# ChuhanZhou/News_Recommendation_Model

Hardware: AMD Instinct MI355X
Metric: train impressions/sec (higher is better)
Workload: dtype f32

## Files before the change

### include/nrm_hotpath.h

```cpp
#ifndef NRM_HOTPATH_H
#define NRM_HOTPATH_H

#ifdef __cplusplus
extern "C" {
#endif

#define NRM_ABI_VERSION 7
#define NRM_OK 0
#define NRM_EINVAL (-1)
#define NRM_ELAUNCH (-2)

typedef void* nrm_stream_t;

int nrm_abi_version(void);
const char* nrm_last_error(void);
int nrm_build_flags(void);
const char* nrm_source_digest(void);
const char* nrm_build_info(void);


#define NRM_MMA_F32 0
#define NRM_MMA_BF16 1
#define NRM_MMA_BF16X3 2
long nrm_pwattn_packed_floats(int D);
// ... 59 lines not shown
    const float* ws; int nsplit, nj, ldws, ni;
    float* out; long out_istride, out_jstride;
    float* out2; long out2_istride, out2_jstride; float sign2;
    const float* vec; float* vec_out;
} nrm_slab_desc;
int nrm_slab_reduce_multi(const nrm_slab_desc* descs, int n, nrm_stream_t stream);

int nrm_head_fold(const float* w_o1, const float* b_o1, const float* w_m2, const float* b_m2, int P, int Q, int R,
                  float* packed_fwd, float* packed_bwd, float* bias, nrm_stream_t stream);
int nrm_head_fold_bwd(const float* dwp, int ldp, const float* dbp, const float* w_o1, const float* w_m2, const float* b_m2,
                      int P, int Q, int R, float* dw_o1, float* dw_m2, float* db_o1, float* db_m2, nrm_stream_t stream);

int nrm_colreduce(int mode, const float* x, const float* dy, const float* mean, const float* rstd,
                  float* s0, float* s1, int R, int N, int ld, nrm_stream_t stream);
int nrm_bn_finalize(int stage, const float* s, float* out, float* running, int R, int N, float momentum, float eps,
                    nrm_stream_t stream);
int nrm_mul_bwd(const float* dy, int lddy, const float* g, int ldg, const float* e, int lde, float* dg, float* de, int ldo,
                int R, int N, nrm_stream_t stream);
int nrm_bn_apply(const float* x, const float* mean, const float* rstd, const float* gamma, const float* beta,
                 float* y, int R, int N, int ld, nrm_stream_t stream);
int nrm_bn_backward(const float* x, const float* dy, const float* mean, const float* rstd, const float* gamma,
                    const float* s0, const float* s1, const float* add, float* dx, int R, int N, int ld, int training,
                    nrm_stream_t stream);
int nrm_concat_cols(const float* const* srcs, const long* lds, const int* widths, int n, float* out, int ldo, long R,
                    nrm_stream_t stream);

int nrm_pool_bmm(const float* W, long wsb, long wsi, long wsj, const float* X, int ldx, float* out,
                 int B, int I, int J, int D, int accumulate, nrm_stream_t stream);
int nrm_pool_rowdot(const float* g, int ldg, const float* h, float* ds, int B, int T, int H, int D, float* zero_out, int zero_n,
                    nrm_stream_t stream);

int nrm_small_linear_relu_fwd(const void* x, int x_is_f64, const float* weight, const float* bias, float* y, long R, int K, int N, int ldy,
                              nrm_stream_t stream);
int nrm_small_linear_relu_bwd(const void* x, int x_is_f64, const float* weight, const float* bias, const float* dy, int lddy, long R,
                              int K, int N, float* dwb, nrm_stream_t stream);

int nrm_loss_fwd_bwd(const float* out, int out_stride, const void* label, int label_is_f64, const long* user_id, const float* delta,
                     long n_delta, float alpha, int B, int T, float* loss_sum, float* dout, int dout_stride, float* ddelta, int* err,
                     nrm_stream_t stream);

int nrm_adam_step(float* p, float* g, float* m, float* v, long n, float lr, float beta1, float beta2, float eps,
                  float weight_decay, int step, int zero_grad, nrm_stream_t stream);
int nrm_gather_flat(const float* const* srcs, const long* offsets, const long* counts, int n, float* flat, long flat_n,
                    nrm_stream_t stream);
int nrm_adam_step_dev(float* p, float* g, float* m, float* v, long n, float lr, float beta1, float beta2, float eps,
                      float weight_decay, float* state, int zero_grad, nrm_stream_t stream);

int nrm_frontend_fwd(const void* x, int x_is_f64, int nrows, int xcols, int P, int n_sub, int behaviour,
                     const float* cat_tab, int n_cat, int e0, const float* sen_w, const float* sen_b, int e1,
                     const float* type_tab, int n_type, int e2,
                     const float* year_tab, const float* month_tab, const float* day_tab, const float* hour_tab,
                     int n_year, int n_month, int n_day, int n_hour, int e3,
                     float* lab, int ldlab, float* ti, int ldti, int* err, nrm_stream_t stream);
int nrm_frontend_bwd(const void* x, int x_is_f64, int nrows, int xcols, int P, int n_sub, int behaviour,
                     const float* dlab, int lddl, const float* sen_w, const float* sen_b,
                     int n_cat, int e0, int e1, int n_type, int e2, int n_year, int n_month, int n_day, int n_hour, int e3,
                     float* d_cat_tab, float* d_sen_w, float* d_sen_b, float* d_type_tab,
                     float* d_year_tab, float* d_month_tab, float* d_day_tab, float* d_hour_tab, nrm_stream_t stream);

long nrm_frontend_tables_ws_floats(long nrows_total, int n_sub, int e1, int n_type, int e2, int n_year, int n_month, int n_day, int n_hour, int e3);
int nrm_frontend_bwd_tables(const void* x0, int nrows0, int xcols0, int behaviour0, const float* dlab0, int lddl0,
                            const void* x1, int nrows1, int xcols1, int behaviour1, const float* dlab1, int lddl1, int x_is_f64,
                            int P, int n_sub, const float* sen_w, const float* sen_b,
                            int e0, int e1, int n_type, int e2, int n_year, int n_month, int n_day, int n_hour, int e3,
                            float* d_sen_w, float* d_sen_b, float* d_type_tab,
                            float* d_year_tab, float* d_month_tab, float* d_day_tab, float* d_hour_tab, float* ws, nrm_stream_t stream);

long nrm_frontend_cat_ws_ints(int n_cat, long nrows_total, int n_sub);
int nrm_frontend_cat_grad(const void* x0, int nrows0, int xcols0, const float* dlab0, int lddl0,
                          const void* x1, int nrows1, int xcols1, const float* dlab1, int lddl1, int x_is_f64,
                          int P, int n_sub, int n_cat, int e0, float* d_cat_tab, int* ws, nrm_stream_t stream);

int nrm_row_auc(const float* score, const float* label, const int* len, int B, int T, float* auc, int* top1,
                nrm_stream_t stream);

int nrm_ensemble_rank_max_candidates(void);
int nrm_ensemble_rank(const float* const* logits, const long* row_stride, const long* col_stride, int M, const int* empty,
                      const float* label, int B, int T, float* score, int* rank, int* live, float* metrics, nrm_stream_t stream);

int nrm_compact_gather(const void* x_target, int target_cols, int target_is_f64, const void* x_global, int global_cols, int global_is_f64,
                       const int* cand_off, const int* pad_mult, int B, int T, int trim, int N,
                       void* xt_compact, void* xg_compact, int* flag, nrm_stream_t stream);
int nrm_pwattn_fwd_ragged(const float* t, const float* h, const float* u, const float* v, const float* packed_wp,
                          const float* w2, const float* b2, float* s, const int* cand_imp, const int* cand_off,
                          int B, int N, int max_count, int H, int D, int mma, nrm_stream_t stream);
int nrm_pool_bmm_ragged(const float* s, const float* h, float* out, const int* cand_off, int B, int N, int max_count, int H, int D,
                        nrm_stream_t stream);
int nrm_ensemble_rank_ragged(const float* const* logits, const long* col_stride, int M, const int* cand_off, const int* pad_mult, int N,
                             const float* label, int B, int T, float* score, int* rank, int* live, float* metrics, nrm_stream_t stream);

int nrm_history_len(const void* x_history, int cols, int is_f64, int B, int H, int* hist_len, nrm_stream_t stream);
int nrm_history_gather(const void* x_history, int cols, int is_f64, const int* hist_off, int B, int H, int R, int k_max, void* xh_compact,
                       nrm_stream_t stream);
int nrm_history_tiles(const int* cand_imp, const int* cand_off, const int* hist_off, const int* tile_pre, int B, int N, int R, int Mt,
                      void* tile_tab, nrm_stream_t stream);
int nrm_pwattn_fwd_hragged(const float* t, const float* h, const float* u, const float* v, const float* packed_wp,
                           const float* w2, const float* b2, float* s, const int* cand_imp, const int* cand_off, const int* hist_off,
                           const int* tile_pre, const void* tile_tab, int B, int N, int max_count, int R, int Mt, int k_max, int D, int mma,
                           nrm_stream_t stream);
int nrm_pool_bmm_hragged(const float* s, const float* h, float* out, const int* cand_off, const int* hist_off, const int* hist_mult,
                         const int* tile_pre, int B, int N, int max_count, int R, int Mt, int k_max, int D, nrm_stream_t stream);

#define NRM_PWATTN_FWD_FORM_LEN 18
#define NRM_FWD_STREAM 0
#define NRM_FWD_RW_TILE 1
#define NRM_FWD_WALK_BF16 2
// ... 58 lines not shown
```

### news_recommendation_model_amd/csrc/capi.hip

```cpp
#include <stdarg.h>
#include <stdint.h>
#include <stdio.h>
#include <stdlib.h>
#include <vector>

#include "../../include/nrm_hotpath.h"
#include "common.hpp"
#include "pwattn.hpp"
#include "gemm.hpp"
#include "head.hpp"
#include "pool_loss.hpp"
#include "frontend.hpp"
#include "scoring.hpp"
#include "compact.hpp"
#include "assemble.hpp"
#include "epoch.hpp"

static thread_local char g_err[512] = "";

static int fail(int code, const char* fmt, ...) {
    va_list ap;
    va_start(ap, fmt);
    vsnprintf(g_err, sizeof(g_err), fmt, ap);
    va_end(ap);
// ... 831 lines not shown
    nrm::EnsembleLogits lg = {};
    for (int m = 0; m < M; ++m) {
        if (!logits[m] && N > 0) return fail(NRM_EINVAL, "nrm_ensemble_rank_ragged: logits[%d] is a null pointer", m);
        const long cs = col_stride ? col_stride[m] : 1;
        if (cs < 1) return fail(NRM_EINVAL, "nrm_ensemble_rank_ragged: model %d has entry stride %ld (need >= 1)", m, cs);
        lg.ptr[m] = logits[m]; lg.row_stride[m] = 0; lg.col_stride[m] = cs;
    }
    return check_hip(nrm::ensemble_rank_ragged_launch(lg, M, cand_off, pad_mult, N, label, B, T, score, rank, live, metrics, (hipStream_t)stream),
                     "ensemble_rank_ragged");
}

int nrm_compact_gather(const void* x_target, int target_cols, int target_is_f64, const void* x_global, int global_cols, int global_is_f64,
                       const int* cand_off, const int* pad_mult, int B, int T, int trim, int N,
                       void* xt_compact, void* xg_compact, int* flag, nrm_stream_t stream) {
    if (B < 0 || T <= 0 || trim < 0 || trim > T || N < 0 || target_cols <= 0 || global_cols <= 0)
        return fail(NRM_EINVAL, "nrm_compact_gather: B=%d T=%d trim=%d N=%d target_cols=%d global_cols=%d", B, T, trim, N, target_cols, global_cols);
    if ((long)N > (long)B * (T - trim)) return fail(NRM_EINVAL, "nrm_compact_gather: N=%d compact rows exceed the B*(T - trim)=%ld kept cells", N, (long)B * (T - trim));
    if (!cand_off || !pad_mult || !flag || !x_target || !x_global || (N > 0 && (!xt_compact || !xg_compact))) return fail(NRM_EINVAL, "nrm_compact_gather: null pointer");
    nrm::CompactGatherParams p;
    p.xt = (const unsigned*)x_target; p.xg = (const unsigned*)x_global; p.xt_c = (unsigned*)xt_compact; p.xg_c = (unsigned*)xg_compact;
    p.wt = target_cols * (target_is_f64 ? 2 : 1); p.wg = global_cols * (global_is_f64 ? 2 : 1);
    p.cand_off = cand_off; p.pad_mult = pad_mult; p.B = B; p.T = T; p.Tp = T - trim; p.N = N; p.flag = flag;
    return check_hip(nrm::compact_gather_launch(p, (hipStream_t)stream), "compact_gather");
}

static int check_fe(const char* fn, int nrows, int xcols, int P, int n_sub, int behaviour, int e0, int e1, int e2, int e3) {
    if (nrows < 0 || P <= 0 || n_sub < 0 || e0 <= 0 || e1 <= 0 || e2 <= 0 || e3 <= 0)
        return fail(NRM_EINVAL, "%s: bad dimension", fn);
    if (n_sub > 16) return fail(NRM_EINVAL, "%s: n_sub=%d (<= 16 sub-category slots)", fn, n_sub);
    const int need = 4 + P + 1 + n_sub + 3 + 1 + (behaviour ? 2 : 0);
    if (xcols < need) return fail(NRM_EINVAL, "%s: packed rows have %d columns, layout needs %d", fn, xcols, need);
    return NRM_OK;
}

int nrm_frontend_fwd(const void* x, int x_is_f64, int nrows, int xcols, int P, int n_sub, int behaviour,
                     const float* cat_tab, int n_cat, int e0, const float* sen_w, const float* sen_b, int e1,
                     const float* type_tab, int n_type, int e2,
                     const float* year_tab, const float* month_tab, const float* day_tab, const float* hour_tab,
                     int n_year, int n_month, int n_day, int n_hour, int e3,
                     float* lab, int ldlab, float* ti, int ldti, int* err, nrm_stream_t stream) {
    if (int rc = check_fe("nrm_frontend_fwd", nrows, xcols, P, n_sub, behaviour, e0, e1, e2, e3)) return rc;
    if (!x || !cat_tab || !sen_w || !sen_b || !type_tab || !year_tab || !month_tab || !day_tab || !hour_tab || !lab || !ti || !err)
        return fail(NRM_EINVAL, "nrm_frontend_fwd: null pointer");
    if (ldlab < e0 + e1 + e2 + e3 + (behaviour ? 2 : 0) || ldti < P) return fail(NRM_EINVAL, "nrm_frontend_fwd: ldlab=%d ldti=%d too small", ldlab, ldti);
    nrm::FrontendParams p = {};
    p.cat_tab = cat_tab; p.sen_w = sen_w; p.sen_b = sen_b; p.type_tab = type_tab;
    p.year_tab = year_tab; p.month_tab = month_tab; p.day_tab = day_tab; p.hour_tab = hour_tab;
    p.n_cat = n_cat; p.n_type = n_type; p.n_year = n_year; p.n_month = n_month; p.n_day = n_day; p.n_hour = n_hour;
    p.e0 = e0; p.e1 = e1; p.e2 = e2; p.e3 = e3; p.P = P; p.n_sub = n_sub; p.xcols = xcols; p.behaviour = behaviour;
    p.lab = lab; p.ldlab = ldlab; p.ti = ti; p.ldti = ldti; p.err = err;
    return check_hip(nrm::frontend_fwd_launch(p, x, x_is_f64, nrows, (hipStream_t)stream), "frontend_fwd");
}

int nrm_frontend_bwd(const void* x, int x_is_f64, int nrows, int xcols, int P, int n_sub, int behaviour,
                     const float* dlab, int lddl, const float* sen_w, const float* sen_b,
                     int n_cat, int e0, int e1, int n_type, int e2, int n_year, int n_month, int n_day, int n_hour, int e3,
                     float* d_cat_tab, float* d_sen_w, float* d_sen_b, float* d_type_tab,
                     float* d_year_tab, float* d_month_tab, float* d_day_tab, float* d_hour_tab, nrm_stream_t stream) {
    if (int rc = check_fe("nrm_frontend_bwd", nrows, xcols, P, n_sub, behaviour, e0, e1, e2, e3)) return rc;
    const int n_small = !!d_sen_w + !!d_sen_b + !!d_type_tab + !!d_year_tab + !!d_month_tab + !!d_day_tab + !!d_hour_tab;
    if (!x || !dlab || !sen_w || !sen_b || (n_small != 7 && (n_small != 0 || !d_cat_tab)))
        return fail(NRM_EINVAL, "nrm_frontend_bwd: null pointer");
    if (lddl < e0 + e1 + e2 + e3) return fail(NRM_EINVAL, "nrm_frontend_bwd: lddl=%d too small", lddl);
    nrm::FrontendParams p = {};
    p.sen_w = sen_w; p.sen_b = sen_b;
    p.d_cat_tab = d_cat_tab; p.d_sen_w = d_sen_w; p.d_sen_b = d_sen_b; p.d_type_tab = d_type_tab;
    p.d_year_tab = d_year_tab; p.d_month_tab = d_month_tab; p.d_day_tab = d_day_tab; p.d_hour_tab = d_hour_tab;
    p.n_cat = n_cat; p.n_type = n_type; p.n_year = n_year; p.n_month = n_month; p.n_day = n_day; p.n_hour = n_hour;
    p.e0 = e0; p.e1 = e1; p.e2 = e2; p.e3 = e3; p.P = P; p.n_sub = n_sub; p.xcols = xcols; p.behaviour = behaviour;
    return check_hip(nrm::frontend_bwd_launch(p, x, x_is_f64, dlab, lddl, nrows, (hipStream_t)stream), "frontend_bwd");
}

static nrm::FrontendParams tab_dims(int n_sub, int e1, int n_type, int e2, int n_year, int n_month, int n_day, int n_hour, int e3) {
    nrm::FrontendParams p = {};
    p.n_type = n_type; p.n_year = n_year; p.n_month = n_month; p.n_day = n_day; p.n_hour = n_hour;
    p.e1 = e1; p.e2 = e2; p.e3 = e3; p.n_sub = n_sub;
    return p;
}

long nrm_frontend_tables_ws_floats(long nrows_total, int n_sub, int e1, int n_type, int e2, int n_year, int n_month, int n_day, int n_hour, int e3) {
    if (nrows_total <= 0 || n_sub < 0) return 0;
    return nrm::tab_grad_ws_floats(tab_dims(n_sub, e1, n_type, e2, n_year, n_month, n_day, n_hour, e3), nrows_total);
}

int nrm_frontend_bwd_tables(const void* x0, int nrows0, int xcols0, int behaviour0, const float* dlab0, int lddl0,
                            const void* x1, int nrows1, int xcols1, int behaviour1, const float* dlab1, int lddl1, int x_is_f64,
                            int P, int n_sub, const float* sen_w, const float* sen_b,
                            int e0, int e1, int n_type, int e2, int n_year, int n_month, int n_day, int n_hour, int e3,
                            float* d_sen_w, float* d_sen_b, float* d_type_tab,
                            float* d_year_tab, float* d_month_tab, float* d_day_tab, float* d_hour_tab, float* ws, nrm_stream_t stream) {
    if (nrows0 > 0) if (int rc = check_fe("nrm_frontend_bwd_tables", nrows0, xcols0, P, n_sub, behaviour0, e0, e1, e2, e3)) return rc;
    if (nrows1 > 0) if (int rc = check_fe("nrm_frontend_bwd_tables", nrows1, xcols1, P, n_sub, behaviour1, e0, e1, e2, e3)) return rc;
    if (nrows0 < 0 || nrows1 < 0 || (long)nrows0 + nrows1 >= (1L << 31) - 64) return fail(NRM_EINVAL, "nrm_frontend_bwd_tables: nrows=%d,%d", nrows0, nrows1);
    if ((nrows0 > 0 && (!x0 || !dlab0 || lddl0 < e0 + e1 + e2 + e3)) || (nrows1 > 0 && (!x1 || !dlab1 || lddl1 < e0 + e1 + e2 + e3)))
        return fail(NRM_EINVAL, "nrm_frontend_bwd_tables: null pointer or lddl too small");
    if (!sen_w || !sen_b || !d_sen_w || !d_sen_b || !d_type_tab || !d_year_tab || !d_month_tab || !d_day_tab || !d_hour_tab || !ws)
        return fail(NRM_EINVAL, "nrm_frontend_bwd_tables: null pointer");
    nrm::FrontendParams p = tab_dims(n_sub, e1, n_type, e2, n_year, n_month, n_day, n_hour, e3);
    p.e0 = e0; p.P = P; p.n_cat = 1;
    p.sen_w = sen_w; p.sen_b = sen_b;
    p.d_sen_w = d_sen_w; p.d_sen_b = d_sen_b; p.d_type_tab = d_type_tab;
    p.d_year_tab = d_year_tab; p.d_month_tab = d_month_tab; p.d_day_tab = d_day_tab; p.d_hour_tab = d_hour_tab;
    if (nrm::tab_grad_ws_floats(p, (long)nrows0 + nrows1) <= 0 && nrows0 + nrows1 > 0)
        return fail(NRM_EINVAL, "nrm_frontend_bwd_tables: shape not taken (nrm_frontend_tables_ws_floats is 0): use nrm_frontend_bwd");
    return check_hip(nrm::tab_grad_launch(p, x0, nrows0, xcols0, dlab0, lddl0, x1, nrows1, xcols1, dlab1, lddl1, x_is_f64, ws,
                                          (hipStream_t)stream), "frontend_bwd_tables");
// ... 101 lines not shown
```

### news_recommendation_model_amd/csrc/frontend.hip

```cpp
#include <algorithm>
#include "common.hpp"
#include "frontend.hpp"

namespace nrm {

template <typename XT>
__device__ __forceinline__ int row_index(const XT* xr, int col, int limit, int* err) {
    const int i = (int)xr[col];
    if (i < 0 || i >= limit) { *err = 1; return i < 0 ? 0 : limit - 1; }
    return i;
}

constexpr int FE_MAXSUB = 16;
constexpr int FE_HDR = 6 + FE_MAXSUB;
struct RowHeaders {
    int* idx;
    float* sen;
};

template <typename XT>
__device__ __forceinline__ void stage_headers(const FrontendParams& p, int xcols, int* err, const XT* __restrict__ x, int r_lo, int nr,
                                              const RowHeaders& hd, int nthreads) {
    const int P = p.P, NS = p.n_sub;
    const int c_cat = 4 + P, c_sub = c_cat + 1, c_sen = c_sub + NS, c_typ = c_sen + 3;
    const int items = 9 + NS;
    for (int i = threadIdx.x; i < nr * items; i += nthreads) {
        const int r = i / items, k = i - r * items;
        const XT* xr = x + (size_t)(r_lo + r) * xcols;
        if (k < 4) {
            const int lim = k == 0 ? p.n_year : k == 1 ? p.n_month : k == 2 ? p.n_day : p.n_hour;
            hd.idx[r * FE_HDR + k] = row_index(xr, k, lim, err);
        } else if (k == 4) {
            hd.idx[r * FE_HDR + 4] = row_index(xr, c_cat, p.n_cat, err);
        } else if (k == 5) {
            hd.idx[r * FE_HDR + 5] = row_index(xr, c_typ, p.n_type, err);
        } else if (k < 6 + NS) {
            hd.idx[r * FE_HDR + k] = row_index(xr, c_sub + (k - 6), p.n_cat, err);
        } else {
            hd.sen[r * 4 + (k - 6 - NS)] = (float)xr[c_sen + (k - 6 - NS)];
        }
    }
}

constexpr int FWD_ROWS = 8;
constexpr int FE_THREADS = 256;

template <typename XT>
__global__ __launch_bounds__(FE_THREADS) void frontend_fwd_kernel(const FrontendParams p, const XT* __restrict__ x, int nrows) {
    __shared__ int h_idx[FWD_ROWS * FE_HDR];
    __shared__ float h_sen[FWD_ROWS * 4];
    const int r_lo = blockIdx.x * FWD_ROWS, nr = min(FWD_ROWS, nrows - r_lo);
    const RowHeaders hd = {h_idx, h_sen};
    stage_headers(p, p.xcols, p.err, x, r_lo, nr, hd, FE_THREADS);
    __syncthreads();
    const int P = p.P, NS = p.n_sub;
    const int c_beh = 4 + P + 1 + NS + 3 + 1;
    const int e0 = p.e0, e1 = p.e1, e2 = p.e2, e3 = p.e3;
    const int width = e0 + e1 + e2 + e3 + (p.behaviour ? 2 : 0);
    const float inv_ns = 1.0f / (float)NS;
    float* lab = p.lab + (size_t)r_lo * p.ldlab;
    for (int i = threadIdx.x; i < nr * p.ldlab; i += FE_THREADS) {
        const int r = i / p.ldlab, c = i - r * p.ldlab;
        const int* hi = h_idx + r * FE_HDR;
        float v = 0.f;
        if (c < e0) {
            float sub = 0.f;
            for (int k = 0; k < NS; ++k) sub += p.cat_tab[(size_t)hi[6 + k] * e0 + c];
            v = p.cat_tab[(size_t)hi[4] * e0 + c] + sub * inv_ns;
        } else if (c < e0 + e1) {
            const int j = c - e0;
            const float pre = p.sen_b[j] + p.sen_w[j * 3] * h_sen[r * 4] + p.sen_w[j * 3 + 1] * h_sen[r * 4 + 1] + p.sen_w[j * 3 + 2] * h_sen[r * 4 + 2];
            v = fmaxf(pre, 0.f);
        } else if (c < e0 + e1 + e2) {
            v = p.type_tab[(size_t)hi[5] * e2 + (c - e0 - e1)];
        } else if (c < e0 + e1 + e2 + e3) {
            const int k = c - e0 - e1 - e2;
            v = p.year_tab[(size_t)hi[0] * e3 + k] + p.month_tab[(size_t)hi[1] * e3 + k] + p.day_tab[(size_t)hi[2] * e3 + k] + p.hour_tab[(size_t)hi[3] * e3 + k];
        } else if (c < width) {
            v = (float)x[(size_t)(r_lo + r) * p.xcols + c_beh + (c - (e0 + e1 + e2 + e3))];
        }
        lab[i] = v;
    }
    float* ti = p.ti + (size_t)r_lo * p.ldti;
    for (int i = threadIdx.x; i < nr * p.ldti; i += FE_THREADS) {
        const int r = i / p.ldti, c = i - r * p.ldti;
        ti[i] = c < P ? (float)x[(size_t)(r_lo + r) * p.xcols + 4 + c] : 0.f;
    }
}

constexpr int FE_ROWS = 32;
constexpr int FE_MAX_BLOCKS = 512;

template <typename XT>
__global__ __launch_bounds__(FE_THREADS) void frontend_bwd_kernel(const FrontendParams p, const XT* __restrict__ x,
                                                                 const float* __restrict__ dlab, int lddl, int nrows) {
    extern __shared__ float sm[];
    const int e0 = p.e0, e1 = p.e1, e2 = p.e2, e3 = p.e3;
    float* a_type = sm;
    float* a_year = a_type + p.n_type * e2;
    float* a_month = a_year + p.n_year * e3;
    float* a_day = a_month + p.n_month * e3;
    float* a_hour = a_day + p.n_day * e3;
    float* a_sen = a_hour + p.n_hour * e3;
    const int total = (int)(a_sen + e1 * 4 - sm);
    const RowHeaders hd = {reinterpret_cast<int*>(sm + total), sm + total + FE_ROWS * FE_HDR};
    for (int i = threadIdx.x; i < total; i += FE_THREADS) sm[i] = 0.f;
    int dummy = 0;
    const int NS = p.n_sub;
    const float inv_ns = 1.0f / (float)NS;
    const int small = e1 + e2 + e3;
    const int ngroups = (nrows + FE_ROWS - 1) / FE_ROWS;
    for (int grp = blockIdx.x; grp < ngroups; grp += gridDim.x) {
        const int r_lo = grp * FE_ROWS, nr = min(FE_ROWS, nrows - r_lo);
        __syncthreads();
        stage_headers(p, p.xcols, &dummy, x, r_lo, nr, hd, FE_THREADS);
        __syncthreads();
        const float* g0 = dlab + (size_t)r_lo * lddl;
        for (int i = threadIdx.x; i < (p.d_cat_tab ? nr * e0 : 0); i += FE_THREADS) {
            const int r = i / e0, c = i - r * e0;
            const int* hi = hd.idx + r * FE_HDR;
            const float gv = g0[(size_t)r * lddl + c];
            atomicAdd(p.d_cat_tab + (size_t)hi[4] * e0 + c, gv);
            const float gs = gv * inv_ns;
            for (int k = 0; k < NS; ++k) atomicAdd(p.d_cat_tab + (size_t)hi[6 + k] * e0 + c, gs);
        }
        for (int i = threadIdx.x; i < (p.d_type_tab ? nr * small : 0); i += FE_THREADS) {
            const int r = i / small, cs = i - r * small;
            const float gv = g0[(size_t)r * lddl + e0 + cs];
            const int* hi = hd.idx + r * FE_HDR;
            if (cs < e1) {
                const float s0 = hd.sen[r * 4], s1 = hd.sen[r * 4 + 1], s2 = hd.sen[r * 4 + 2];
                const float pre = p.sen_b[cs] + p.sen_w[cs * 3] * s0 + p.sen_w[cs * 3 + 1] * s1 + p.sen_w[cs * 3 + 2] * s2;
                if (pre > 0.f && gv != 0.f) {
                    atomicAdd(a_sen + cs * 4 + 0, gv * s0);
                    atomicAdd(a_sen + cs * 4 + 1, gv * s1);
                    atomicAdd(a_sen + cs * 4 + 2, gv * s2);
                    atomicAdd(a_sen + cs * 4 + 3, gv);
                }
            } else if (cs < e1 + e2) {
                atomicAdd(a_type + hi[5] * e2 + (cs - e1), gv);
            } else {
                const int k = cs - e1 - e2;
                atomicAdd(a_year + hi[0] * e3 + k, gv);
                atomicAdd(a_month + hi[1] * e3 + k, gv);
                atomicAdd(a_day + hi[2] * e3 + k, gv);
                atomicAdd(a_hour + hi[3] * e3 + k, gv);
            }
        }
    }
    __syncthreads();
    if (!p.d_type_tab) return;
    for (int i = threadIdx.x; i < p.n_type * e2; i += FE_THREADS) if (a_type[i] != 0.f) atomicAdd(p.d_type_tab + i, a_type[i]);
    for (int i = threadIdx.x; i < p.n_year * e3; i += FE_THREADS) if (a_year[i] != 0.f) atomicAdd(p.d_year_tab + i, a_year[i]);
    for (int i = threadIdx.x; i < p.n_month * e3; i += FE_THREADS) if (a_month[i] != 0.f) atomicAdd(p.d_month_tab + i, a_month[i]);
    for (int i = threadIdx.x; i < p.n_day * e3; i += FE_THREADS) if (a_day[i] != 0.f) atomicAdd(p.d_day_tab + i, a_day[i]);
    for (int i = threadIdx.x; i < p.n_hour * e3; i += FE_THREADS) if (a_hour[i] != 0.f) atomicAdd(p.d_hour_tab + i, a_hour[i]);
    for (int i = threadIdx.x; i < e1 * 4; i += FE_THREADS) {
        const float v = a_sen[i];
        if (v != 0.f) {
            const int j = i >> 2, w = i & 3;
            if (w < 3) atomicAdd(p.d_sen_w + j * 3 + w, v); else atomicAdd(p.d_sen_b + j, v);
        }
    }
}

static size_t bwd_lds_bytes(const FrontendParams& p) {
    return sizeof(float) * ((size_t)p.n_type * p.e2 + (size_t)(p.n_year + p.n_month + p.n_day + p.n_hour) * p.e3 + (size_t)p.e1 * 4 +
                            (size_t)FE_ROWS * (FE_HDR + 4));
}

hipError_t frontend_fwd_launch(const FrontendParams& p, const void* x, int x_is_f64, int nrows, hipStream_t st) {
    if (nrows <= 0) return hipSuccess;
    if (p.n_sub > FE_MAXSUB) return hipErrorInvalidValue;
    const dim3 grid((nrows + FWD_ROWS - 1) / FWD_ROWS);
    if (x_is_f64) hipLaunchKernelGGL(frontend_fwd_kernel<double>, grid, dim3(FE_THREADS), 0, st, p, (const double*)x, nrows);
    else          hipLaunchKernelGGL(frontend_fwd_kernel<float>, grid, dim3(FE_THREADS), 0, st, p, (const float*)x, nrows);
    return hipGetLastError();
}

hipError_t frontend_bwd_launch(const FrontendParams& p, const void* x, int x_is_f64, const float* dlab, int lddl,
                               int nrows, hipStream_t st) {
    if (nrows <= 0) return hipSuccess;
    const size_t shm = bwd_lds_bytes(p);
    if (shm > 160 * 1024 || p.n_sub > FE_MAXSUB) return hipErrorInvalidValue;
    const dim3 grid(std::min((nrows + FE_ROWS - 1) / FE_ROWS, FE_MAX_BLOCKS));
    if (x_is_f64) {
        if (shm > 64 * 1024) { hipError_t e = hipFuncSetAttribute((const void*)frontend_bwd_kernel<double>, hipFuncAttributeMaxDynamicSharedMemorySize, (int)shm); if (e != hipSuccess) return e; }
        hipLaunchKernelGGL(frontend_bwd_kernel<double>, grid, dim3(FE_THREADS), shm, st, p, (const double*)x, dlab, lddl, nrows);
    } else {
        if (shm > 64 * 1024) { hipError_t e = hipFuncSetAttribute((const void*)frontend_bwd_kernel<float>, hipFuncAttributeMaxDynamicSharedMemorySize, (int)shm); if (e != hipSuccess) return e; }
        hipLaunchKernelGGL(frontend_bwd_kernel<float>, grid, dim3(FE_THREADS), shm, st, p, (const float*)x, dlab, lddl, nrows);
    }
    return hipGetLastError();
}

constexpr int TB_THREADS = 512;
constexpr int TB_WAVES = TB_THREADS / 64;
constexpr int TB_ROWS = 32;
constexpr int TB_MAXT = 16;
constexpr int TB_MAXTILES = TB_WAVES * TB_MAXT;
constexpr int TB_WG_PER_CU = 2;
constexpr int TB_CB = 4;
constexpr int TB_RED_CELLS = 64, TB_RED_SLICES = 16;

struct TabTile {
    short hdr, ibase;
    short coff, ncol;
    int dst;
    short ldr, ldc;
};
struct TabSet { const void* x; const float* dlab; int nrows, xcols, lddl, nchunks; };
struct TabParams {
    FrontendParams p;
    TabSet set[2];
    int ntiles, tiles_per_wave, cells, ldb, chunks_per_wg;
    float* ws;
    TabTile tile[TB_MAXTILES];
};

__device__ __forceinline__ bool fe_finite(float v) { return fabsf(v) <= 3.402823466e+38f; }

template <typename XT, int NT>
__global__ __launch_bounds__(TB_THREADS, TB_WG_PER_CU * TB_WAVES / 4) void tab_grad_kernel(const TabParams q) {
    extern __shared__ float sm[];
    const FrontendParams& p = q.p;
    const int e0 = p.e0, e1 = p.e1, e2 = p.e2, e3 = p.e3;
    const int small = e1 + e2 + e3, ldb = q.ldb;
    float* s_b = sm;
    float* s_wb = s_b + TB_ROWS * ldb;
// ... 474 lines not shown
```

### news_recommendation_model_amd/csrc/frontend.hpp

```cpp
#pragma once
#include <hip/hip_runtime.h>

namespace nrm {
struct FrontendParams {
    const float *cat_tab, *sen_w, *sen_b, *type_tab, *year_tab, *month_tab, *day_tab, *hour_tab;
    float *d_cat_tab, *d_sen_w, *d_sen_b, *d_type_tab, *d_year_tab, *d_month_tab, *d_day_tab, *d_hour_tab;
    int n_cat, n_type, n_year, n_month, n_day, n_hour;
    int e0, e1, e2, e3;
    int P, n_sub, xcols, behaviour;
    float* lab; int ldlab;
    float* ti; int ldti;
    int* err;
};
hipError_t frontend_fwd_launch(const FrontendParams& p, const void* x, int x_is_f64, int nrows, hipStream_t st);
hipError_t frontend_bwd_launch(const FrontendParams& p, const void* x, int x_is_f64, const float* dlab, int lddl,
                               int nrows, hipStream_t st);
long tab_grad_ws_floats(const FrontendParams& p, long nrows_total);
hipError_t tab_grad_launch(const FrontendParams& p, const void* x0, int nrows0, int xcols0, const float* dlab0, int lddl0,
                           const void* x1, int nrows1, int xcols1, const float* dlab1, int lddl1, int x_is_f64, float* ws, hipStream_t st);
long cat_grad_ws_ints(int n_cat, long nrows_total, int n_sub);
hipError_t cat_grad_launch(const void* x0, int nrows0, int xcols0, const float* dlab0, int lddl0,
                           const void* x1, int nrows1, int xcols1, const float* dlab1, int lddl1, int x_is_f64,
                           int P, int n_sub, int n_cat, int e0, float* d_cat, int* ws, hipStream_t st);
}
```

### news_recommendation_model_amd/native.py

```python
from __future__ import annotations

import ctypes
import os
import threading

_HERE = os.path.dirname(os.path.abspath(__file__))
LIB_PATH = os.environ.get("NRM_HOTPATH_LIB") or os.path.join(_HERE, "libnrm_hotpath.so")
ABI_VERSION = 7

_c_fp = ctypes.c_void_p
_c_i, _c_l = ctypes.c_int, ctypes.c_long

SIGNATURES = {
    "nrm_abi_version": (_c_i, []),
    "nrm_last_error": (ctypes.c_char_p, []),
    "nrm_build_flags": (_c_i, []),
    "nrm_source_digest": (ctypes.c_char_p, []),
    "nrm_build_info": (ctypes.c_char_p, []),
    "nrm_pwattn_packed_floats": (_c_l, [_c_i]),
    "nrm_pwattn_pack_wp": (_c_i, [_c_fp, _c_i, _c_i, _c_i, _c_fp, _c_fp]),
    "nrm_pwattn_fwd": (_c_i, [_c_fp] * 9 + [_c_i] * 5 + [_c_fp]),
    "nrm_pwattn_bwd_dz": (_c_i, [_c_fp] * 7 + [_c_i] * 5 + [_c_fp]),
    "nrm_pwattn_bwd_rw_supported": (_c_i, [_c_i, _c_i]),
    "nrm_pwattn_bwd_rw_packed_floats": (_c_l, [_c_i, _c_i]),
# ... 15 lines not shown
    "nrm_gemm_nt": (_c_i, [_c_fp, _c_i, _c_i, _c_fp, _c_i, _c_i, _c_fp, _c_fp, _c_i, _c_fp, _c_i, _c_fp, _c_i, _c_i, _c_i, _c_fp]),
    "nrm_slab_reduce": (_c_i, [_c_fp, _c_i, _c_i, _c_i, _c_i, _c_fp, _c_l, _c_l, _c_fp, _c_l, _c_l, ctypes.c_float,
                               _c_fp, _c_fp, _c_fp]),
    "nrm_bn_finalize": (_c_i, [_c_i, _c_fp, _c_fp, _c_fp, _c_i, _c_i, ctypes.c_float, ctypes.c_float, _c_fp]),
    "nrm_mul_bwd": (_c_i, [_c_fp, _c_i, _c_fp, _c_i, _c_fp, _c_i, _c_fp, _c_fp, _c_i, _c_i, _c_i, _c_fp]),
    "nrm_gemm_tn_nsplit": (_c_i, [_c_i, _c_i, _c_i, _c_i]),
    "nrm_gemm_tn": (_c_i, [_c_fp, _c_i, _c_i, _c_fp, _c_i, _c_i, _c_i, _c_fp, _c_i, _c_fp, _c_fp, _c_l, _c_i, _c_fp]),
    "nrm_gemm_pack_multi": (_c_i, [_c_fp, _c_i, _c_fp]),
    "nrm_slab_reduce_multi": (_c_i, [_c_fp, _c_i, _c_fp]),
    "nrm_head_fold": (_c_i, [_c_fp] * 4 + [_c_i] * 3 + [_c_fp] * 4),
    "nrm_head_fold_bwd": (_c_i, [_c_fp, _c_i, _c_fp, _c_fp, _c_fp, _c_fp, _c_i, _c_i, _c_i] + [_c_fp] * 5),
    "nrm_colreduce": (_c_i, [_c_i] + [_c_fp] * 6 + [_c_i] * 3 + [_c_fp]),
    "nrm_bn_apply": (_c_i, [_c_fp] * 6 + [_c_i] * 3 + [_c_fp]),
    "nrm_bn_backward": (_c_i, [_c_fp] * 9 + [_c_i] * 4 + [_c_fp]),
    "nrm_concat_cols": (_c_i, [_c_fp, _c_fp, _c_fp, _c_i, _c_fp, _c_i, _c_l, _c_fp]),
    "nrm_pool_bmm": (_c_i, [_c_fp, _c_l, _c_l, _c_l, _c_fp, _c_i, _c_fp] + [_c_i] * 5 + [_c_fp]),
    "nrm_pool_rowdot": (_c_i, [_c_fp, _c_i, _c_fp, _c_fp] + [_c_i] * 4 + [_c_fp, _c_i, _c_fp]),
    "nrm_small_linear_relu_fwd": (_c_i, [_c_fp, _c_i, _c_fp, _c_fp, _c_fp, _c_l, _c_i, _c_i, _c_i, _c_fp]),
    "nrm_small_linear_relu_bwd": (_c_i, [_c_fp, _c_i, _c_fp, _c_fp, _c_fp, _c_i, _c_l, _c_i, _c_i, _c_fp, _c_fp]),
    "nrm_loss_fwd_bwd": (_c_i, [_c_fp, _c_i, _c_fp, _c_i, _c_fp, _c_fp, _c_l, ctypes.c_float, _c_i, _c_i, _c_fp, _c_fp, _c_i, _c_fp, _c_fp, _c_fp]),
    "nrm_adam_step": (_c_i, [_c_fp] * 4 + [_c_l] + [ctypes.c_float] * 5 + [_c_i, _c_i, _c_fp]),
    "nrm_adam_step_dev": (_c_i, [_c_fp] * 4 + [_c_l] + [ctypes.c_float] * 5 + [_c_fp, _c_i, _c_fp]),
    "nrm_gather_flat": (_c_i, [_c_fp, _c_fp, _c_fp, _c_i, _c_fp, _c_l, _c_fp]),
    "nrm_row_auc": (_c_i, [_c_fp] * 3 + [_c_i, _c_i] + [_c_fp] * 3),
    "nrm_ensemble_rank_max_candidates": (_c_i, []),
    "nrm_ensemble_rank": (_c_i, [_c_fp] * 3 + [_c_i, _c_fp, _c_fp, _c_i, _c_i] + [_c_fp] * 5),
    "nrm_compact_gather": (_c_i, [_c_fp, _c_i, _c_i, _c_fp, _c_i, _c_i, _c_fp, _c_fp, _c_i, _c_i, _c_i, _c_i, _c_fp, _c_fp, _c_fp, _c_fp]),
    "nrm_pwattn_fwd_ragged": (_c_i, [_c_fp] * 10 + [_c_i] * 6 + [_c_fp]),
    "nrm_pool_bmm_ragged": (_c_i, [_c_fp] * 4 + [_c_i] * 5 + [_c_fp]),
    "nrm_history_len": (_c_i, [_c_fp, _c_i, _c_i, _c_i, _c_i, _c_fp, _c_fp]),
    "nrm_history_gather": (_c_i, [_c_fp, _c_i, _c_i, _c_fp, _c_i, _c_i, _c_i, _c_i, _c_fp, _c_fp]),
    "nrm_history_tiles": (_c_i, [_c_fp] * 4 + [_c_i] * 4 + [_c_fp, _c_fp]),
    "nrm_pwattn_fwd_hragged": (_c_i, [_c_fp] * 13 + [_c_i] * 8 + [_c_fp]),
    "nrm_pwattn_fwd_form": (_c_i, [_c_i] * 11 + [ctypes.POINTER(ctypes.c_int)]),
    "nrm_pool_bmm_hragged": (_c_i, [_c_fp] * 7 + [_c_i] * 7 + [_c_fp]),
    "nrm_history_gather_groups": (_c_i, [_c_fp, _c_i, _c_i] + [_c_fp] * 4 + [_c_i] * 4 + [_c_fp, _c_fp]),
    "nrm_pool_bmm_wlast": (_c_i, [_c_fp, _c_l, _c_l, _c_l, _c_fp, _c_i, _c_fp] + [_c_i] * 5 + [ctypes.c_float, _c_i, _c_fp]),
    "nrm_pool_rowdot_wlast": (_c_i, [_c_fp, _c_i, _c_fp, _c_fp] + [_c_i] * 4 + [_c_fp, _c_i, ctypes.c_float, _c_fp]),
    "nrm_candidate_gather_groups": (_c_i, [_c_fp, _c_i, _c_i, _c_fp, _c_i, _c_i, _c_fp, _c_i] + [_c_fp] * 4 + [_c_i] * 4 + [_c_fp] * 6),
    "nrm_colreduce_roww": (_c_i, [_c_i] + [_c_fp] * 4 + [_c_i] * 3 + [_c_fp]),
    "nrm_bn_backward_roww": (_c_i, [_c_fp] * 10 + [_c_i] * 4 + [_c_fp]),
    "nrm_loss_fwd_bwd_wlast": (_c_i, [_c_fp, _c_i, _c_fp, _c_i, _c_fp, _c_fp, _c_l, ctypes.c_float, _c_i, _c_i, ctypes.c_float, ctypes.c_float,
                                      _c_fp, _c_fp, _c_i, _c_fp, _c_fp, _c_fp]),
    "nrm_ensemble_rank_ragged": (_c_i, [_c_fp, _c_fp, _c_i, _c_fp, _c_fp, _c_i, _c_fp, _c_i, _c_i] + [_c_fp] * 5),
    "nrm_assemble_batch": (_c_i, [_c_fp, _c_fp, _c_i, _c_i, _c_i, _c_i, _c_fp]),
    "nrm_assemble_form": (_c_i, [_c_i, _c_i]),
    "nrm_assemble_batch_at": (_c_i, [_c_fp, _c_fp, _c_l, _c_fp, _c_i, _c_i, _c_i, _c_i, _c_fp]),
    "nrm_assemble_groups_at": (_c_i, [_c_fp, _c_fp, _c_fp, _c_l, _c_fp, _c_i, _c_i, _c_i, _c_i, _c_fp]),
    "nrm_epoch_tally": (_c_i, [_c_fp, _c_fp, _c_fp, _c_i, _c_fp, _c_fp, _c_fp, _c_fp, _c_l, _c_fp]),
    "nrm_eval_tally": (_c_i, [_c_fp] * 6 + [_c_i] * 3 + [_c_fp, _c_l] + [_c_fp] * 5 + [_c_l, _c_fp]),
    "nrm_frontend_fwd": (_c_i, [_c_fp, _c_i, _c_i, _c_i, _c_i, _c_i, _c_i,  _c_fp, _c_i, _c_i,  _c_fp, _c_fp, _c_i,
                                 _c_fp, _c_i, _c_i,  _c_fp, _c_fp, _c_fp, _c_fp,  _c_i, _c_i, _c_i, _c_i, _c_i,
                                 _c_fp, _c_i, _c_fp, _c_i, _c_fp, _c_fp]),
    "nrm_frontend_tables_ws_floats": (_c_l, [_c_l] + [_c_i] * 9),
    "nrm_frontend_bwd_tables": (_c_i, [_c_fp, _c_i, _c_i, _c_i, _c_fp, _c_i] * 2 + [_c_i] * 3 + [_c_fp, _c_fp] + [_c_i] * 9
                                + [_c_fp] * 8 + [_c_fp]),
    "nrm_frontend_cat_ws_ints": (_c_l, [_c_i, _c_l, _c_i]),
    "nrm_frontend_cat_grad": (_c_i, [_c_fp, _c_i, _c_i, _c_fp, _c_i] * 2 + [_c_i] * 5 + [_c_fp, _c_fp, _c_fp]),
    "nrm_frontend_bwd": (_c_i, [_c_fp, _c_i, _c_i, _c_i, _c_i, _c_i, _c_i,  _c_fp, _c_i, _c_fp, _c_fp]
                         + [_c_i] * 10 + [_c_fp] * 8 + [_c_fp]),
}



class PackDesc(ctypes.Structure):
    _fields_ = [("src", ctypes.c_void_p), ("src2", ctypes.c_void_p), ("sign2", ctypes.c_float),
                ("row_stride", ctypes.c_long), ("col_stride", ctypes.c_long), ("nrows", ctypes.c_int), ("ncols", ctypes.c_int),
                ("packed", ctypes.c_void_p), ("mma", ctypes.c_int)]


class SlabDesc(ctypes.Structure):
    _fields_ = [("ws", ctypes.c_void_p), ("nsplit", ctypes.c_int), ("nj", ctypes.c_int), ("ldws", ctypes.c_int), ("ni", ctypes.c_int),
                ("out", ctypes.c_void_p), ("out_istride", ctypes.c_long), ("out_jstride", ctypes.c_long),
                ("out2", ctypes.c_void_p), ("out2_istride", ctypes.c_long), ("out2_jstride", ctypes.c_long), ("sign2", ctypes.c_float),
                ("vec", ctypes.c_void_p), ("vec_out", ctypes.c_void_p)]


class AssembleTables(ctypes.Structure):
    _fields_ = ([(n, ctypes.c_void_p) for n in ("art_static", "art_global", "art_pub_us", "art_id", "user_off", "ev_art", "ev_time_us", "ev_read",
                                                "ev_scroll", "user_id", "imp_user", "imp_time_us", "imp_off", "imp_inview", "imp_target", "imp_id")]
                + [(n, ctypes.c_long) for n in ("A", "U", "E", "N", "L")]
                + [(n, ctypes.c_int) for n in ("S", "static_cols", "is_f64")]
                + [(n, ctypes.c_void_p) for n in ("x_history", "x_target", "x_global", "label", "label_id", "empty_num", "user_id_out",
                                                  "impression_id", "history_len", "err")])


class AssembleGroups(ctypes.Structure):
    _fields_ = ([(n, ctypes.c_void_p) for n in ("bounds", "h_g", "hist_row_off", "t_g", "cand_row_off")]
                + [(n, ctypes.c_int) for n in ("G", "R", "N")]
                + [(n, ctypes.c_void_p) for n in ("label_arena", "row_weight", "misfit")])


_lib = None
_lock = threading.Lock()


def load():
    global _lib
    if _lib is not None:
        return _lib
    with _lock:
        if _lib is not None:
            return _lib
        if not os.path.exists(LIB_PATH):
            raise RuntimeError(
                f"{LIB_PATH} is missing: build it with `python -m news_recommendation_model_amd.build` "
# ... 55 lines not shown
```

Before: 36280.

## Vectorize frontend forward kernel with quad loads, nontemporal stores, specialized templates

Rewrites the frontend forward kernel so each thread handles four consecutive columns. Table gathers and input row reads use 16-byte vector loads chosen at runtime from pointer alignment, and outputs use nontemporal vector stores. The ti copy is unrolled and moved ahead of the barrier, and templates are specialised on load width and on n_sub=5. This cuts per-element index arithmetic and scalar memory traffic in an embedding-gather stage, at the cost of more template instances and more complex alignment-dependent code paths.

```diff
diff --git a/include/nrm_hotpath.h b/include/nrm_hotpath.h
--- a/include/nrm_hotpath.h
+++ b/include/nrm_hotpath.h
@@ -135,6 +135,7 @@
                      const float* year_tab, const float* month_tab, const float* day_tab, const float* hour_tab,
                      int n_year, int n_month, int n_day, int n_hour, int e3,
                      float* lab, int ldlab, float* ti, int ldti, int* err, nrm_stream_t stream);
+int nrm_frontend_load_width(const void* x, int x_is_f64, int xcols, int P);
 int nrm_frontend_bwd(const void* x, int x_is_f64, int nrows, int xcols, int P, int n_sub, int behaviour,
                      const float* dlab, int lddl, const float* sen_w, const float* sen_b,
                      int n_cat, int e0, int e1, int n_type, int e2, int n_year, int n_month, int n_day, int n_hour, int e3,
diff --git a/news_recommendation_model_amd/csrc/capi.hip b/news_recommendation_model_amd/csrc/capi.hip
--- a/news_recommendation_model_amd/csrc/capi.hip
+++ b/news_recommendation_model_amd/csrc/capi.hip
@@ -907,6 +907,11 @@
     return check_hip(nrm::frontend_fwd_launch(p, x, x_is_f64, nrows, (hipStream_t)stream), "frontend_fwd");
 }
 
+int nrm_frontend_load_width(const void* x, int x_is_f64, int xcols, int P) {
+    if (xcols <= 0 || P <= 0) return fail(NRM_EINVAL, "nrm_frontend_load_width: xcols=%d P=%d", xcols, P);
+    return nrm::frontend_load_width(x, x_is_f64, xcols, P);
+}
+
 int nrm_frontend_bwd(const void* x, int x_is_f64, int nrows, int xcols, int P, int n_sub, int behaviour,
                      const float* dlab, int lddl, const float* sen_w, const float* sen_b,
                      int n_cat, int e0, int e1, int n_type, int e2, int n_year, int n_month, int n_day, int n_hour, int e3,
diff --git a/news_recommendation_model_amd/csrc/frontend.hip b/news_recommendation_model_amd/csrc/frontend.hip
--- a/news_recommendation_model_amd/csrc/frontend.hip
+++ b/news_recommendation_model_amd/csrc/frontend.hip
@@ -43,48 +43,194 @@
 }
 
 constexpr int FWD_ROWS = 8;
+constexpr int FWD_UNROLL = 4;
 constexpr int FE_THREADS = 256;
 
+struct FwdForm { int cat, sen, type, time, lab_vec, ti_vec; };
+
+int frontend_load_width(const void* x, int x_is_f64, int xcols, int P) {
+    const uintptr_t a = reinterpret_cast<uintptr_t>(x);
+    const size_t pitch = (size_t)xcols * (x_is_f64 ? 8 : 4);
+    if (P < 4) return 1;
+    if (a % 16 == 0 && pitch % 16 == 0) return 4;
+    if (!x_is_f64 && a % 8 == 0 && pitch % 8 == 0) return 2;
+    return 1;
+}
+
+static int quad_class(const float* base, int e, int first) {
+    const uintptr_t a = reinterpret_cast<uintptr_t>(base);
+    if (a % 16 == 0 && e % 4 == 0 && first % 4 == 0) return 2;
+    if (a % 8 == 0 && e % 2 == 0 && first % 2 == 0) return 1;
+    return 0;
+}
+
+__device__ __forceinline__ f32x4 load_quad(const float* __restrict__ q, int cls) {
+    if (cls == 2) return *reinterpret_cast<const f32x4*>(q);
+    if (cls == 1) {
+        const f32x2 lo = *reinterpret_cast<const f32x2*>(q), hi = *reinterpret_cast<const f32x2*>(q + 2);
+        return f32x4{lo[0], lo[1], hi[0], hi[1]};
+    }
+    return f32x4{q[0], q[1], q[2], q[3]};
+}
+
+template <typename XT, int LW>
+__device__ __forceinline__ f32x4 load_row_quad(const XT* __restrict__ s) {
+    if constexpr (sizeof(XT) == 4 && LW == 4) {
+        return *reinterpret_cast<const f32x4*>(s);
+    } else if constexpr (sizeof(XT) == 4 && LW == 2) {
+        const f32x2 lo = *reinterpret_cast<const f32x2*>(s), hi = *reinterpret_cast<const f32x2*>(s + 2);
+        return f32x4{lo[0], lo[1], hi[0], hi[1]};
+    } else if constexpr (sizeof(XT) == 8 && LW == 4) {
+        using f64x2 = __attribute__((ext_vector_type(2))) double;
+        const f64x2 lo = *reinterpret_cast<const f64x2*>(s), hi = *reinterpret_cast<const f64x2*>(s + 2);
+        return f32x4{(float)lo[0], (float)lo[1], (float)hi[0], (float)hi[1]};
+    } else {
+        return f32x4{(float)s[0], (float)s[1], (float)s[2], (float)s[3]};
+    }
+}
+
+struct QuadWalk {
+    int r, cq, nq, dr, dq;
+    __device__ __forceinline__ QuadWalk(int nq_, int start, int step) : nq(nq_) {
+        r = start / nq; cq = start - r * nq;
+        dr = step / nq; dq = step - dr * nq;
+    }
+    __device__ __forceinline__ void next() {
+        r += dr; cq += dq;
+        if (cq >= nq) { cq -= nq; ++r; }
+    }
+};
+
 template <typename XT>
-__global__ __launch_bounds__(FE_THREADS) void frontend_fwd_kernel(const FrontendParams p, const XT* __restrict__ x, int nrows) {
+__device__ __forceinline__ float label_element(const FrontendParams& p, const XT* __restrict__ xr, const int* hi, const float* hs, int c) {
+    const int e0 = p.e0, e1 = p.e1, e2 = p.e2, e3 = p.e3, NS = p.n_sub;
+    const int width = e0 + e1 + e2 + e3 + (p.behaviour ? 2 : 0);
+    float v = 0.f;
+    if (c < e0) {
+        const float inv_ns = 1.0f / (float)NS;
+        float sub = 0.f;
+        for (int k = 0; k < NS; ++k) sub += p.cat_tab[(size_t)hi[6 + k] * e0 + c];
+        v = p.cat_tab[(size_t)hi[4] * e0 + c] + sub * inv_ns;
+    } else if (c < e0 + e1) {
+        const int j = c - e0;
+        const float pre = p.sen_b[j] + p.sen_w[j * 3] * hs[0] + p.sen_w[j * 3 + 1] * hs[1] + p.sen_w[j * 3 + 2] * hs[2];
+        v = fmaxf(pre, 0.f);
+    } else if (c < e0 + e1 + e2) {
+        v = p.type_tab[(size_t)hi[5] * e2 + (c - e0 - e1)];
+    } else if (c < e0 + e1 + e2 + e3) {
+        const int k = c - e0 - e1 - e2;
+        v = p.year_tab[(size_t)hi[0] * e3 + k] + p.month_tab[(size_t)hi[1] * e3 + k] + p.day_tab[(size_t)hi[2] * e3 + k] + p.hour_tab[(size_t)hi[3] * e3 + k];
+    } else if (c < width) {
+        v = (float)xr[4 + p.P + 1 + NS + 3 + 1 + (c - (e0 + e1 + e2 + e3))];
+    }
+    return v;
+}
+
+template <typename XT, int LW, int NSC>
+__global__ __launch_bounds__(FE_THREADS) void frontend_fwd_kernel(const FrontendParams p, const FwdForm f, const XT* __restrict__ x, int nrows) {
     __shared__ int h_idx[FWD_ROWS * FE_HDR];
     __shared__ float h_sen[FWD_ROWS * 4];
     const int r_lo = blockIdx.x * FWD_ROWS, nr = min(FWD_ROWS, nrows - r_lo);
     const RowHeaders hd = {h_idx, h_sen};
     stage_headers(p, p.xcols, p.err, x, r_lo, nr, hd, FE_THREADS);
+    const int P = p.P, NS = NSC ? NSC : p.n_sub;
+    constexpr int NSB = NSC ? NSC : 4;
+    const XT* __restrict__ xw = x + (size_t)r_lo * p.xcols;
+
+    {
+        float* __restrict__ ti = p.ti + (size_t)r_lo * p.ldti;
+        const int ldti = p.ldti;
+        QuadWalk w((ldti + 3) >> 2, threadIdx.x, FE_THREADS);
+        while (w.r < nr) {
+            int rr[FWD_UNROLL], cc[FWD_UNROLL];
+            f32x4 v[FWD_UNROLL];
+#pragma unroll
+            for (int u = 0; u < FWD_UNROLL; ++u) {
+                rr[u] = w.r; cc[u] = 4 * w.cq;
+                w.next();
+                v[u] = f32x4{0.f, 0.f, 0.f, 0.f};
+                if (rr[u] < nr) {
+                    const XT* __restrict__ s = xw + (size_t)rr[u] * p.xcols + 4 + cc[u];
+                    if (cc[u] + 4 <= P) {
+                        v[u] = load_row_quad<XT, LW>(s);
+                    } else {
+#pragma unroll
+                        for (int k = 0; k < 4; ++k) if (cc[u] + k < P) v[u][k] = (float)s[k];
+                    }
+                }
+            }
+#pragma unroll
+            for (int u = 0; u < FWD_UNROLL; ++u) {
+                if (rr[u] >= nr) break;
+                float* d = ti + (size_t)rr[u] * ldti + cc[u];
+                if (f.ti_vec) {
+                    __builtin_nontemporal_store(v[u], reinterpret_cast<f32x4*>(d));
+                } else {
+#pragma unroll
+                    for (int k = 0; k < 4; ++k) if (cc[u] + k < ldti) d[k] = v[u][k];
+                }
+            }
+        }
+    }
     __syncthreads();
-    const int P = p.P, NS = p.n_sub;
-    const int c_beh = 4 + P + 1 + NS + 3 + 1;
-    const int e0 = p.e0, e1 = p.e1, e2 = p.e2, e3 = p.e3;
-    const int width = e0 + e1 + e2 + e3 + (p.behaviour ? 2 : 0);
+
+    const int e0 = p.e0, e1 = p.e1, e2 = p.e2, e3 = p.e3, ldlab = p.ldlab;
+    const int o1 = e0 + e1, o2 = o1 + e2, o3 = o2 + e3;
     const float inv_ns = 1.0f / (float)NS;
-    float* lab = p.lab + (size_t)r_lo * p.ldlab;
-    for (int i = threadIdx.x; i < nr * p.ldlab; i += FE_THREADS) {
-        const int r = i / p.ldlab, c = i - r * p.ldlab;
+    float* __restrict__ lab = p.lab + (size_t)r_lo * ldlab;
+    for (QuadWalk w((ldlab + 3) >> 2, threadIdx.x, FE_THREADS); w.r < nr; w.next()) {
+        const int r = w.r, c = 4 * w.cq;
         const int* hi = h_idx + r * FE_HDR;
-        float v = 0.f;
-        if (c < e0) {
-            float sub = 0.f;
-            for (int k = 0; k < NS; ++k) sub += p.cat_tab[(size_t)hi[6 + k] * e0 + c];
-            v = p.cat_tab[(size_t)hi[4] * e0 + c] + sub * inv_ns;
-        } else if (c < e0 + e1) {
-            const int j = c - e0;
-            const float pre = p.sen_b[j] + p.sen_w[j * 3] * h_sen[r * 4] + p.sen_w[j * 3 + 1] * h_sen[r * 4 + 1] + p.sen_w[j * 3 + 2] * h_sen[r * 4 + 2];
-            v = fmaxf(pre, 0.f);
-        } else if (c < e0 + e1 + e2) {
-            v = p.type_tab[(size_t)hi[5] * e2 + (c - e0 - e1)];
-        } else if (c < e0 + e1 + e2 + e3) {
-            const int k = c - e0 - e1 - e2;
-            v = p.year_tab[(size_t)hi[0] * e3 + k] + p.month_tab[(size_t)hi[1] * e3 + k] + p.day_tab[(size_t)hi[2] * e3 + k] + p.hour_tab[(size_t)hi[3] * e3 + k];
-        } else if (c < width) {
-            v = (float)x[(size_t)(r_lo + r) * p.xcols + c_beh + (c - (e0 + e1 + e2 + e3))];
-        }
-        lab[i] = v;
-    }
-    float* ti = p.ti + (size_t)r_lo * p.ldti;
-    for (int i = threadIdx.x; i < nr * p.ldti; i += FE_THREADS) {
-        const int r = i / p.ldti, c = i - r * p.ldti;
-        ti[i] = c < P ? (float)x[(size_t)(r_lo + r) * p.xcols + 4 + c] : 0.f;
+        const float* hs = h_sen + r * 4;
+        f32x4 v;
+        if (c + 4 <= e0) {
+            const f32x4 cv = load_quad(p.cat_tab + (size_t)hi[4] * e0 + c, f.cat);
+            f32x4 sub = f32x4{0.f, 0.f, 0.f, 0.f};
+            for (int k0 = 0; k0 < NS; k0 += NSB) {
+                f32x4 sv[NSB];
+#pragma unroll
+                for (int u = 0; u < NSB; ++u)
+                    if (k0 + u < NS) sv[u] = load_quad(p.cat_tab + (size_t)hi[6 + k0 + u] * e0 + c, f.cat);
+#pragma unroll
+                for (int u = 0; u < NSB; ++u)
+                    if (k0 + u < NS) {
+#pragma unroll
+                        for (int j = 0; j < 4; ++j) sub[j] += sv[u][j];
+                    }
+            }
+#pragma unroll
+            for (int j = 0; j < 4; ++j) v[j] = cv[j] + sub[j] * inv_ns;
+        } else if (c >= e0 && c + 4 <= o1 && f.sen == 2) {
+            const int j0 = c - e0;
+            const f32x4 b = load_quad(p.sen_b + j0, 2);
+            f32x4 wq[3];
+#pragma unroll
+            for (int k = 0; k < 3; ++k) wq[k] = load_quad(p.sen_w + 3 * j0 + 4 * k, 2);
+#pragma unroll
+            for (int j = 0; j < 4; ++j) {
+                const float pre = b[j] + wq[(3 * j) >> 2][(3 * j) & 3] * hs[0] + wq[(3 * j + 1) >> 2][(3 * j + 1) & 3] * hs[1] + wq[(3 * j + 2) >> 2][(3 * j + 2) & 3] * hs[2];
+                v[j] = fmaxf(pre, 0.f);
+            }
+        } else if (c >= o1 && c + 4 <= o2) {
+            v = load_quad(p.type_tab + (size_t)hi[5] * e2 + (c - o1), f.type);
+        } else if (c >= o2 && c + 4 <= o3) {
+            const int k = c - o2;
+            const f32x4 ty = load_quad(p.year_tab + (size_t)hi[0] * e3 + k, f.time), tm = load_quad(p.month_tab + (size_t)hi[1] * e3 + k, f.time);
+            const f32x4 td = load_quad(p.day_tab + (size_t)hi[2] * e3 + k, f.time), th = load_quad(p.hour_tab + (size_t)hi[3] * e3 + k, f.time);
+#pragma unroll
+            for (int j = 0; j < 4; ++j) v[j] = ty[j] + tm[j] + td[j] + th[j];
+        } else {
+            const XT* __restrict__ xr = xw + (size_t)r * p.xcols;
+#pragma unroll
+            for (int j = 0; j < 4; ++j) v[j] = label_element(p, xr, hi, hs, c + j);
+        }
+        float* d = lab + (size_t)r * ldlab + c;
+        if (f.lab_vec) {
+            __builtin_nontemporal_store(v, reinterpret_cast<f32x4*>(d));
+        } else {
+#pragma unroll
+            for (int j = 0; j < 4; ++j) if (c + j < ldlab) d[j] = v[j];
+        }
     }
 }
 
@@ -172,9 +318,29 @@
 hipError_t frontend_fwd_launch(const FrontendParams& p, const void* x, int x_is_f64, int nrows, hipStream_t st) {
     if (nrows <= 0) return hipSuccess;
     if (p.n_sub > FE_MAXSUB) return hipErrorInvalidValue;
+    auto aligned16 = [](const void* q) { return reinterpret_cast<uintptr_t>(q) % 16 == 0; };
+    FwdForm f;
+    f.cat = quad_class(p.cat_tab, p.e0, 0);
+    f.sen = aligned16(p.sen_b) && aligned16(p.sen_w) && p.e0 % 4 == 0 ? 2 : 0;
+    f.type = quad_class(p.type_tab, p.e2, p.e0 + p.e1);
+    f.time = std::min(std::min(quad_class(p.year_tab, p.e3, p.e0 + p.e1 + p.e2), quad_class(p.month_tab, p.e3, p.e0 + p.e1 + p.e2)),
+                      std::min(quad_class(p.day_tab, p.e3, p.e0 + p.e1 + p.e2), quad_class(p.hour_tab, p.e3, p.e0 + p.e1 + p.e2)));
+    f.lab_vec = aligned16(p.lab) && p.ldlab % 4 == 0;
+    f.ti_vec = aligned16(p.ti) && p.ldti % 4 == 0;
+    const int lw = frontend_load_width(x, x_is_f64, p.xcols, p.P);
     const dim3 grid((nrows + FWD_ROWS - 1) / FWD_ROWS);
-    if (x_is_f64) hipLaunchKernelGGL(frontend_fwd_kernel<double>, grid, dim3(FE_THREADS), 0, st, p, (const double*)x, nrows);
-    else          hipLaunchKernelGGL(frontend_fwd_kernel<float>, grid, dim3(FE_THREADS), 0, st, p, (const float*)x, nrows);
+    auto launch = [&](auto kernel, auto* xt) { hipLaunchKernelGGL(kernel, grid, dim3(FE_THREADS), 0, st, p, f, xt, nrows); };
+    const bool ns5 = p.n_sub == 5;
+    if (x_is_f64) {
+        const double* xd = (const double*)x;
+        if (lw == 4) ns5 ? launch(frontend_fwd_kernel<double, 4, 5>, xd) : launch(frontend_fwd_kernel<double, 4, 0>, xd);
+        else         ns5 ? launch(frontend_fwd_kernel<double, 1, 5>, xd) : launch(frontend_fwd_kernel<double, 1, 0>, xd);
+    } else {
+        const float* xf = (const float*)x;
+        if (lw == 4)      ns5 ? launch(frontend_fwd_kernel<float, 4, 5>, xf) : launch(frontend_fwd_kernel<float, 4, 0>, xf);
+        else if (lw == 2) ns5 ? launch(frontend_fwd_kernel<float, 2, 5>, xf) : launch(frontend_fwd_kernel<float, 2, 0>, xf);
+        else              ns5 ? launch(frontend_fwd_kernel<float, 1, 5>, xf) : launch(frontend_fwd_kernel<float, 1, 0>, xf);
+    }
     return hipGetLastError();
 }
 
diff --git a/news_recommendation_model_amd/csrc/frontend.hpp b/news_recommendation_model_amd/csrc/frontend.hpp
--- a/news_recommendation_model_amd/csrc/frontend.hpp
+++ b/news_recommendation_model_amd/csrc/frontend.hpp
@@ -13,6 +13,7 @@
     int* err;
 };
 hipError_t frontend_fwd_launch(const FrontendParams& p, const void* x, int x_is_f64, int nrows, hipStream_t st);
+int frontend_load_width(const void* x, int x_is_f64, int xcols, int P);
 hipError_t frontend_bwd_launch(const FrontendParams& p, const void* x, int x_is_f64, const float* dlab, int lddl,
                                int nrows, hipStream_t st);
 long tab_grad_ws_floats(const FrontendParams& p, long nrows_total);
diff --git a/news_recommendation_model_amd/native.py b/news_recommendation_model_amd/native.py
--- a/news_recommendation_model_amd/native.py
+++ b/news_recommendation_model_amd/native.py
@@ -91,6 +91,7 @@
     "nrm_frontend_fwd": (_c_i, [_c_fp, _c_i, _c_i, _c_i, _c_i, _c_i, _c_i,  _c_fp, _c_i, _c_i,  _c_fp, _c_fp, _c_i,
                                  _c_fp, _c_i, _c_i,  _c_fp, _c_fp, _c_fp, _c_fp,  _c_i, _c_i, _c_i, _c_i, _c_i,
                                  _c_fp, _c_i, _c_fp, _c_i, _c_fp, _c_fp]),
+    "nrm_frontend_load_width": (_c_i, [_c_fp, _c_i, _c_i, _c_i]),
     "nrm_frontend_tables_ws_floats": (_c_l, [_c_l] + [_c_i] * 9),
     "nrm_frontend_bwd_tables": (_c_i, [_c_fp, _c_i, _c_i, _c_i, _c_fp, _c_i] * 2 + [_c_i] * 3 + [_c_fp, _c_fp] + [_c_i] * 9
                                 + [_c_fp] * 8 + [_c_fp]),
```

Result: no change. 36390, median of 6 (+0.3%).
